# nirvanesque/headCT_foundation

Measured on AMD Instinct MI355X. Metric: CT-volumes/sec MAE pretrain step (96^3, ViT-B/16^3, mask 0.75), higher is better.
Workload: dtype bf16; 1 GPU; BASELINE config #2: MAE ViT-B/16^3, 96^3x1ch, mask 0.75, full train step (fwd+bwd+clip+AdamW+LR); per_gpu_batch=256, global_batch=256, parallelism=dp1, init=reference init, seed 42

## Files before the change

### headct_foundation_amd/_lib.py

```python
from __future__ import annotations

import ctypes as C
import os
from typing import Optional

HERE = os.path.dirname(os.path.abspath(__file__))
LIB_PATH = os.path.join(HERE, "libheadct_hip.so")

HCT_F32, HCT_BF16, HCT_F16 = 0, 1, 2
NORM_LAYERNORM, NORM_RMSNORM = 0, 1
HCT_ACT_NONE, HCT_ACT_GELU, HCT_ACT_DGELU, HCT_ACT_TANH, HCT_ACT_GELU_D, HCT_ACT_MULAUX = 0, 1, 2, 3, 4, 5
ACT_NONE, ACT_GELU, ACT_DGELU = 0, 1, 2

c_void_p, c_int, c_float, c_size_t, c_int64 = C.c_void_p, C.c_int, C.c_float, C.c_size_t, C.c_int64


class GemmArgs(C.Structure):
    _fields_ = [
        ("M", c_int), ("N", c_int), ("K", c_int),
        ("A", c_void_p), ("a_dtype", c_int), ("lda", c_int64), ("transA", c_int),
        ("B", c_void_p), ("b_dtype", c_int), ("ldb", c_int64), ("transB", c_int),
        ("C", c_void_p), ("c_dtype", c_int), ("ldc", c_int64),
        ("bias", c_void_p), ("residual", c_void_p), ("ldr", c_int64),
        ("act", c_int),
# ... 135 lines not shown
    "hct_adjust_contrast_workspace_bytes": (c_size_t, [c_int, c_int64]),
    "hct_adjust_contrast": (c_int, [c_void_p, c_int, c_int64, c_void_p, c_void_p, c_void_p, c_size_t, c_void_p]),
    "hct_volume_to_ras": (c_int, [c_void_p, c_int, c_int, c_int, c_int, C.POINTER(c_int), C.POINTER(c_int), c_int, C.c_double, C.c_double,
                                  c_void_p, c_void_p]),
    "hct_bspline3_resample_workspace_bytes": (c_size_t, [c_int] * 6),
    "hct_bspline3_resample": (c_int, [c_void_p, c_int, c_int, c_int, c_void_p, c_int, c_int, c_int, c_void_p, c_void_p, c_void_p, c_size_t, c_void_p]),
    "hct_foreground_bbox_workspace_bytes": (c_size_t, [c_int] * 3),
    "hct_foreground_bbox": (c_int, [c_void_p, c_int, c_int, c_int, c_void_p, c_void_p, c_void_p, c_size_t, c_void_p]),
    "hct_crop_window_resize_area": (c_int, [c_void_p, c_int, c_int, c_int, c_void_p, c_int, c_void_p, c_void_p, c_void_p, c_int, c_int, c_int,
                                            c_void_p]),
    "hct_pos_embed_interp3d": (c_int, [c_void_p, c_int, c_void_p, c_int, c_int, c_int, c_void_p]),
    "hct_colsum_workspace_bytes": (c_size_t, [c_int, c_int]),
    "hct_colsum": (c_int, [c_void_p, c_int, c_int, c_int, c_int64, c_void_p, c_void_p, c_size_t, c_void_p]),
    "hct_cast": (c_int, [c_void_p, c_int, c_void_p, c_int, c_int64, c_void_p]),
    "hct_transpose_cast": (c_int, [c_void_p, c_int, c_void_p, c_int, c_int, c_int, c_void_p]),
    "hct_grad_norms_workspace_bytes": (c_size_t, [c_int64]),
    "hct_grad_norms": (c_int, [c_void_p, c_void_p, c_int, c_int64, c_float, c_int, c_void_p, c_void_p, c_void_p, c_size_t, c_void_p]),
    "hct_adamw_step": (c_int, [c_void_p, c_void_p, c_void_p, c_void_p, c_void_p, c_void_p, c_void_p, c_int, c_int64, c_float, c_float,
                               c_float, c_float, c_float, c_int, c_void_p, c_void_p]),
    "hct_lion_step": (c_int, [c_void_p] * 6 + [c_int, c_int64] + [C.c_double] * 4 + [c_void_p, c_void_p]),
    "hct_sgd_step": (c_int, [c_void_p] * 6 + [c_int, c_int64] + [C.c_double] * 2 + [c_void_p, c_void_p]),
    "hct_lamb_workspace_bytes": (c_size_t, [c_int64, c_int]),
    "hct_lamb_step": (c_int, [c_void_p] * 7 + [c_int, c_int64] + [C.c_double] * 5 + [c_void_p] * 4 + [c_size_t, c_void_p, c_void_p]),
    "hct_debug_set_gemm_variant": (None, [c_int]),
    "hct_gemm_nt_stream_k_bytes": (c_size_t, []),
    "hct_gemm_tn_group_workspace_bytes": (c_size_t, [c_int]),
    "hct_gemm_tn_group_prepare": (c_int, [c_void_p, c_int, c_void_p, c_size_t, c_void_p]),
    "hct_gemm_tn_group_run": (c_int, [c_void_p, c_int, c_void_p, c_size_t, c_void_p]),
    "hct_prof_enable": (None, [c_int]),
    "hct_prof_reset": (None, []),
    "hct_prof_read": (c_int, [c_int, C.POINTER(C.c_double), C.POINTER(c_int64), C.POINTER(C.c_double)]),
    "hct_prof_read_bytes": (c_int, [c_int, C.POINTER(C.c_double)]),
    "hct_prof_shapes": (c_int, [c_int, c_void_p, c_int]),
    "hct_mae_plan_create": (c_void_p, [C.POINTER(MaeConfig), c_int, c_int]),
# ... 9 lines not shown
    "hct_mae_backward_final_offset": (c_int64, [c_void_p]),
    "hct_mae_plan_set_wgrad_defer": (c_int, [c_void_p, c_int, c_int]),
    "hct_mae_plan_set_requires_grad": (c_int, [c_void_p, c_int, c_int]),
    "hct_lora_qv_fwd": (c_int, [c_void_p, c_void_p, c_void_p, c_void_p, c_void_p, c_int, c_int, c_int, c_int, c_int, c_int, c_void_p, c_void_p, c_void_p]),
    "hct_lora_qv_bwd_workspace_bytes": (c_size_t, [c_int, c_int, c_int, c_int]),
    "hct_lora_qv_bwd": (c_int, [c_void_p] * 11 + [c_int] * 6 + [c_void_p] * 6 + [c_size_t, c_void_p]),
    "hct_topk_dot_chunks": (c_int, [c_int, c_int64]),
    "hct_topk_dot_workspace": (c_size_t, [c_int, c_int64, c_int]),
    "hct_topk_dot": (c_int, [c_void_p, c_int, c_void_p, c_int64, c_int, c_int, c_void_p, c_int, c_void_p, c_void_p, c_void_p, c_size_t, c_void_p]),
    "hct_attention_row_probs": (c_int, [c_void_p, c_int, c_int, c_int, c_int, c_int, c_void_p, c_int, c_void_p, c_void_p]),
    "hct_mae_recon_accum": (c_int, [c_void_p, c_int, c_int, c_void_p, c_int, c_void_p, c_int, c_int, c_int, c_int, c_int, c_void_p, c_void_p, c_void_p,
                                    c_void_p]),
    "hct_mae_recon_finish": (c_int, [c_void_p, c_void_p, c_void_p, c_void_p, c_int, c_int, c_int, c_int, c_int, c_void_p, c_void_p, c_void_p, c_void_p]),
    "hct_mae_plan_bind": (c_int, [c_void_p, c_void_p, c_void_p, c_void_p, c_void_p, c_void_p, c_size_t]),
    "hct_mae_refresh_weights": (c_int, [c_void_p, c_int, c_void_p]),
    "hct_mae_forward": (c_int, [c_void_p, c_void_p, c_int, c_void_p, c_void_p, c_float, c_void_p]),
    "hct_mae_set_loss_grad": (c_int, [c_void_p, c_void_p]),
    "hct_mae_num_backward_stages": (c_int, [c_void_p]),
    "hct_mae_backward_stage_range": (c_int, [c_void_p, c_int, C.POINTER(c_int64), C.POINTER(c_int64)]),
    "hct_mae_backward_stage": (c_int, [c_void_p, c_int, c_void_p]),
    "hct_vit_forward": (c_int, [c_void_p, c_void_p, c_int, c_void_p]),
    "hct_vit_forward_parts": (c_int, [c_void_p, C.POINTER(c_void_p), c_int, c_int, c_void_p]),
    "hct_vit_backward_stage": (c_int, [c_void_p, c_int, c_void_p, c_void_p]),
    "hct_vit_assemble_bwd": (c_int, [c_void_p, c_int, c_int, c_int, c_int, c_void_p, c_int, c_void_p, c_void_p, c_void_p, c_void_p]),
    "hct_mae_plan_activation": (c_void_p, [c_void_p, C.c_char_p, C.POINTER(c_int64), C.POINTER(c_int64), C.POINTER(c_int)]),
}

_lib: Optional[C.CDLL] = None


# ... 83 lines not shown
```

### headct_foundation_amd/csrc/mae_plan.hip

```cpp
#include <cstdlib>
#include "common.h"
#include "gemm_plan.h"

#include <algorithm>
#include <map>
#include <string>
#include <vector>

using namespace hct;

namespace {

constexpr int64_t kUnitElems = 1024;

struct BlockP {
  int ln1_w, ln1_b, qkv_w, qkv_b, proj_w, proj_b, ln2_w, ln2_b, fc1_w, fc1_b, fc2_w, fc2_b;
  int lq_b = -1, lq_a = -1, lv_b = -1, lv_a = -1;
  int site = 0;
};
struct BlockA {
  size_t x1, mean1, rstd1, qkv, o, lse, h_mid, x2, mean2, rstd2, u, g;
  size_t lora_t = 0;
};
struct Act { size_t off; int64_t rows, cols; int dtype; };
// ... 8 lines not shown
  int g, L, K, pd, Ne, Nd, Me, Md;
  int D, Dd, Mlp, Mlpd, H, Hd;
  std::vector<hct_param_info> params;
  std::map<std::string, int> pindex;
  int64_t param_elems = 0, bf16t_elems = 0;
  bool vit = false;
  int R = 0;
  int lora = 0;
  int norm_kind = 0;
  float drop_p = 0.f;
  bool drop_on = false;
  bool drop_fwd = false;
  uint64_t drop_seed = 0;
  size_t s_drop_y = 0;
  bool t_all_done = false;
  float norm_eps = 1e-5f;
  int p_reg = -1;
  int p_pe_w, p_pe_b, p_pos, p_cls, p_norm_w, p_norm_b, p_de_w, p_de_b, p_mask, p_dcls, p_dpos, p_dnorm_w, p_dnorm_b,
      p_pred_w, p_pred_b;
  std::vector<BlockP> enc, dec;
  std::vector<std::pair<int64_t, int64_t>> stage_range;
  size_t ws_bytes = 0;
  size_t a_ids_restore, a_ids_shuffle, a_mask, a_row_loss, a_patches, a_tok, a_latent, a_lat_mean, a_lat_rstd, a_e,
      a_ynorm, a_yn_mean, a_yn_rstd, a_pred, a_dpred;
  bool tail = false;
  bool tail_fwd = false;
  bool tail_ok = false;
  int Mc = 0;
  size_t a_tail_rows = 0, a_tail_inv = 0, a_oc = 0, s_dhc = 0;
  bool dec0 = false, dec0_fwd = false, dec0_ok = false;
// ... 799 lines not shown
}

void hct_mae_plan_destroy(hct_mae_plan* p) { delete p; }
int hct_mae_plan_num_params(const hct_mae_plan* p) { return (int)p->params.size(); }
int hct_mae_plan_param_info(const hct_mae_plan* p, int index, hct_param_info* out) {
  HCT_REQUIRE(p && out && index >= 0 && index < (int)p->params.size(), "hct_mae_plan_param_info: bad index");
  *out = p->params[index];
  return 0;
}
int64_t hct_mae_plan_param_elems(const hct_mae_plan* p) { return p->param_elems; }
int64_t hct_mae_plan_bf16_t_elems(const hct_mae_plan* p) { return p->bf16t_elems; }
size_t hct_mae_plan_workspace_bytes(const hct_mae_plan* p) { return p->ws_bytes; }
int hct_mae_plan_len_keep(const hct_mae_plan* p) { return p ? p->K : -1; }
int hct_mae_plan_set_requires_grad(hct_mae_plan* p, int index, int flag) {
  HCT_REQUIRE(p && index >= 0 && index < (int)p->params.size(), "hct_mae_plan_set_requires_grad: bad index");
  if (p->params[index].requires_grad != (flag ? 1 : 0)) p->t_all_done = false;
  p->params[index].requires_grad = flag ? 1 : 0;
  return 0;
}
int hct_mae_plan_set_dec0(hct_mae_plan* p, int on) {
  if (!p) return -1;
  p->dec0 = on != 0 && p->dec0_ok;
  return p->dec0 ? 1 : 0;
}
int hct_mae_plan_set_dropout(hct_mae_plan* p, int active, uint64_t seed) {
  if (!p) return -1;
  p->drop_on = active != 0 && p->drop_p > 0.f;
  p->drop_seed = seed;
  return p->drop_on ? 1 : 0;
}
int hct_mae_plan_set_tail(hct_mae_plan* p, int compact) {
  if (!p) return -1;
  p->tail = compact != 0 && p->tail_ok;
  return p->tail ? 1 : 0;
}

int hct_mae_plan_bind(hct_mae_plan* p, float* params, float* grads, void* params_bf16, void* params_bf16_t, void* workspace,
                      size_t workspace_bytes) {
  HCT_REQUIRE(p && params && workspace, "hct_mae_plan_bind: null buffer");
  HCT_REQUIRE(p->dt == HCT_F32 || (params_bf16 && params_bf16_t), "hct_mae_plan_bind: bf16 mode needs the bf16 weight buffers");
  if (workspace_bytes < p->ws_bytes) { set_error("hct_mae_plan_bind: workspace too small"); return HCT_E_WORKSPACE; }
  p->params_f32 = params; p->grads = grads;
  p->params_bf16 = (bf16*)params_bf16; p->params_bf16_t = (bf16*)params_bf16_t;
  p->ws = (unsigned char*)workspace;
  p->nt_ws_armed = false;
  p->t_all_done = false;
  p->fwd_done = false;
  for (auto& v : p->wg_prepared) v.clear();
  p->wg_pending.clear();
  return 0;
}

int hct_mae_refresh_weights(hct_mae_plan* p, int with_plain, void* stream) {
  HCT_REQUIRE(p && p->params_f32, "hct_mae_refresh_weights: plan not bound");
  if (p->dt != HCT_BF16) return 0;
  if (with_plain) RC(hct_cast(p->params_f32, HCT_F32, p->params_bf16, HCT_BF16, p->param_elems, stream));
  TransposeTable t;
  t.n = 0;
  t.tile_start[0] = 0;
  auto flush = [&]() -> int {
    if (t.n == 0) return 0;
    hipLaunchKernelGGL(transpose_cast_batched_kernel, dim3(t.tile_start[t.n]), dim3(256), 0, (hipStream_t)stream, p->params_f32,
                       p->params_bf16_t, t);
    t.n = 0;
    return check_hip(hipGetLastError(), "hct_mae_refresh_weights");
  };
  for (const auto& pi : p->params) {
    if (pi.bf16_t_offset < 0) continue;
    if (!with_plain && p->t_all_done && !pi.requires_grad) continue;
    const int rows = (int)pi.shape[0], cols = (int)(pi.numel / pi.shape[0]);
    t.rows[t.n] = rows; t.cols[t.n] = cols; t.src[t.n] = pi.offset; t.dst[t.n] = pi.bf16_t_offset;
    t.tile_start[t.n + 1] = t.tile_start[t.n] + ((rows + 63) / 64) * ((cols + 63) / 64);
    if (++t.n == kMaxT) RC(flush());
  }
  RC(flush());
  p->t_all_done = true;
  return 0;
}

int hct_mae_forward(hct_mae_plan* p, const void* x, int x_dtype, const float* noise, float* loss, float grad_scale, void* stream) {
  HCT_REQUIRE(p && p->ws && x && noise && loss, "hct_mae_forward: plan not bound or null argument");
  HCT_REQUIRE(!p->vit, "hct_mae_forward: encoder-only plans are driven by hct_vit_forward");
  HCT_REQUIRE(x_dtype == HCT_F32 || x_dtype == HCT_F16, "hct_mae_forward: volumes are fp32 or fp16");
  hipStream_t s = (hipStream_t)stream;
  unsigned char* ws = p->ws;
  const hct_mae_config& c = p->cfg;
  const int B = p->B;
  int32_t* ids_restore = (int32_t*)(ws + p->a_ids_restore);
  int32_t* ids_shuffle = (int32_t*)(ws + p->a_ids_shuffle);
  float* mask = (float*)(ws + p->a_mask);
// ... 213 lines not shown
```

### headct_foundation_amd/csrc/optim.hip

```cpp
#include "common.h"

namespace hct {

constexpr int kUnit = 1024;

__device__ __forceinline__ float block_sum_256(float v, float* s_tmp) {
  v = wave_sum(v);
  __syncthreads();
  if ((threadIdx.x & 63) == 0) s_tmp[threadIdx.x >> 6] = v;
  __syncthreads();
  return (s_tmp[0] + s_tmp[1]) + (s_tmp[2] + s_tmp[3]);
}

__global__ void __launch_bounds__(256) sumsq_units_kernel(const float* __restrict__ g, int64_t total,
                                                          float* __restrict__ unit_sumsq) {
  __shared__ float s_tmp[4];
  const int64_t i = (int64_t)blockIdx.x * kUnit + threadIdx.x * 4;
  float s = 0.f;
  if (i < total) {
    const f32x4 v = Vec4<float>::load(g + i);
    s = (v[0] * v[0] + v[1] * v[1]) + (v[2] * v[2] + v[3] * v[3]);
  }
  s = block_sum_256(s, s_tmp);
  if (threadIdx.x == 0) unit_sumsq[blockIdx.x] = s;
// ... 33 lines not shown
  const int64_t base = (int64_t)blockIdx.x * kUnit;
  const float c = coef[find_segment(seg_off, nseg, base)];
  if (c == 1.0f) return;
  const int64_t i = base + threadIdx.x * 4;
  if (i < total) Vec4<float>::store(g + i, Vec4<float>::load(g + i) * c);
}

struct AdamArgs {
  float lr_wd_keep;
  float one_m_b1, b2, one_m_b2;
  float step_size;
  float inv_bc2_sqrt;
  float eps;
};

__global__ void __launch_bounds__(256) adamw_units_kernel(float* __restrict__ p, float* __restrict__ g, float* __restrict__ m,
                                                          float* __restrict__ v, const int64_t* __restrict__ seg_off,
                                                          const float* __restrict__ coef, const uint8_t* __restrict__ skip,
                                                          int nseg, int64_t total, AdamArgs a, bf16* __restrict__ p_bf16) {
  const int64_t base = (int64_t)blockIdx.x * kUnit;
  const int sgi = find_segment(seg_off, nseg, base);
  const int64_t i = base + threadIdx.x * 4;
  if (i >= total) return;
  if (skip && skip[sgi]) return;
  const float c = coef ? coef[sgi] : 1.0f;
  f32x4 gv = Vec4<float>::load_nt(g + i);
  if (c != 1.0f) {
    gv = gv * c;
    Vec4<float>::store(g + i, gv);
  }
  f32x4 pv = Vec4<float>::load_nt(p + i) * a.lr_wd_keep;
  f32x4 mv = Vec4<float>::load_nt(m + i);
  mv = mv + (gv - mv) * a.one_m_b1;
  f32x4 vv = Vec4<float>::load_nt(v + i) * a.b2 + gv * gv * a.one_m_b2;
  f32x4 den;
#pragma unroll
  for (int e = 0; e < 4; ++e) den[e] = sqrtf(vv[e]) * a.inv_bc2_sqrt + a.eps;
#pragma unroll
  for (int e = 0; e < 4; ++e) pv[e] = pv[e] - a.step_size * (mv[e] / den[e]);
  Vec4<float>::store_nt(p + i, pv);
  Vec4<float>::store_nt(m + i, mv);
  Vec4<float>::store_nt(v + i, vv);
  if (p_bf16) Vec4<bf16>::store(p_bf16 + i, pv);
}

struct LionArgs {
  float lr_wd_keep;
  float lr, b1, one_m_b1, b2, one_m_b2;
};

__global__ void __launch_bounds__(256) lion_units_kernel(float* __restrict__ p, float* __restrict__ g, float* __restrict__ m,
                                                         const int64_t* __restrict__ seg_off, const float* __restrict__ coef,
                                                         const uint8_t* __restrict__ skip, int nseg, int64_t total, LionArgs a,
                                                         bf16* __restrict__ p_bf16) {
  const int64_t base = (int64_t)blockIdx.x * kUnit;
  const int sgi = find_segment(seg_off, nseg, base);
  const int64_t i = base + threadIdx.x * 4;
  if (i >= total) return;
// ... 141 lines not shown
  HCT_REQUIRE(total > 0 && total % kUnit == 0 && nseg > 0, "hct_grad_norms: total must be a positive multiple of %d", kUnit);
  if (workspace_bytes < hct_grad_norms_workspace_bytes(total)) {
    set_error("hct_grad_norms: workspace too small");
    return HCT_E_WORKSPACE;
  }
  hipStream_t s = (hipStream_t)stream;
  const int units = (int)(total / kUnit);
  hipLaunchKernelGGL(sumsq_units_kernel, dim3(units), dim3(256), 0, s, grads, total, (float*)workspace);
  hipLaunchKernelGGL(seg_norm_kernel, dim3(nseg), dim3(256), 0, s, (const float*)workspace, seg_off, clip, norms, coef);
  if (scale_in_place && clip > 0.f)
    hipLaunchKernelGGL(scale_units_kernel, dim3(units), dim3(256), 0, s, grads, seg_off, coef, nseg, total);
  HCT_CHECK_LAUNCH("hct_grad_norms");
  return 0;
}

int hct_adamw_step(float* params, float* grads, float* exp_avg, float* exp_avg_sq, const int64_t* seg_off,
                   const float* coef, const uint8_t* skip, int nseg, int64_t total, float lr, float beta1, float beta2,
                   float eps, float weight_decay, int step, void* params_bf16, void* stream) {
  HCT_REQUIRE(total > 0 && total % kUnit == 0 && nseg > 0 && step >= 1, "hct_adamw_step: bad arguments");
  AdamArgs a;
  const double bc1 = 1.0 - pow((double)beta1, (double)step);
  const double bc2 = 1.0 - pow((double)beta2, (double)step);
  a.lr_wd_keep = (float)(1.0 - (double)lr * (double)weight_decay);
  a.one_m_b1 = (float)(1.0 - (double)beta1);
  a.b2 = beta2;
  a.one_m_b2 = (float)(1.0 - (double)beta2);
  a.step_size = (float)((double)lr / bc1);
  a.inv_bc2_sqrt = (float)(1.0 / sqrt(bc2));
  a.eps = eps;
  hipLaunchKernelGGL(adamw_units_kernel, dim3((int)(total / kUnit)), dim3(256), 0, (hipStream_t)stream, params, grads,
                     exp_avg, exp_avg_sq, seg_off, coef, skip, nseg, total, a, (bf16*)params_bf16);
  HCT_CHECK_LAUNCH("hct_adamw_step");
  return 0;
}

int hct_lion_step(float* params, float* grads, float* exp_avg, const int64_t* seg_off, const float* coef, const uint8_t* skip,
                  int nseg, int64_t total, double lr, double beta1, double beta2, double weight_decay, void* params_bf16,
                  void* stream) {
  HCT_REQUIRE(params && grads && exp_avg && seg_off && total > 0 && total % kUnit == 0 && nseg > 0, "hct_lion_step: bad arguments");
  LionArgs a;
  a.lr_wd_keep = (float)(1.0 - lr * weight_decay);
  a.lr = (float)lr;
  a.b1 = (float)beta1;
  a.one_m_b1 = (float)(1.0 - beta1);
  a.b2 = (float)beta2;
  a.one_m_b2 = (float)(1.0 - beta2);
  hipLaunchKernelGGL(lion_units_kernel, dim3((int)(total / kUnit)), dim3(256), 0, (hipStream_t)stream, params, grads, exp_avg,
// ... 54 lines not shown
```

### headct_foundation_amd/flat.py

```python
from __future__ import annotations

import ctypes as C
from typing import Callable, Dict, List, Optional, Tuple

import torch
import torch.nn as nn

from . import _lib
from ._lib import HCT_BF16, HctError


class FlatModule(nn.Module):

    def _init_flat(self) -> None:
        self._weights_version = 0
        self._managed_updates = False
        self._grad_prescale = 1.0
        self._build_flat(torch.device("cpu"))

    def _flat_layout(self) -> Tuple[List[Tuple[str, int, int, Tuple[int, ...], bool, int]], int]:
        layout, off = [], 0
        for n, p in self.named_parameters():
            layout.append((n, off, p.numel(), tuple(p.shape), bool(p.requires_grad), -1))
            off += (p.numel() + 1023) // 1024 * 1024
# ... 137 lines not shown
        for name, off, numel, shape, rg, _ in self._layout:
            p = self._named_cache[name]
            p.requires_grad_(rg and p.requires_grad)
            g = old_grads[name]
            if g is not None:
                self._flat_grad[off:off + numel].copy_(g.reshape(-1))
                p.grad = self._flat_grad[off:off + numel].view(shape)
        if self._dt == HCT_BF16:
            self._flat_bf16 = torch.zeros(total, dtype=torch.bfloat16, device=device)
            self._flat_bf16_t = torch.zeros(max(self._bf16_t_elems, 1), dtype=torch.bfloat16, device=device)
        else:
            self._flat_bf16 = self._flat_bf16_t = None
        self._plans = {}
        self._plain_fresh = False

    def mark_weights_updated(self, plain_bf16_fresh: bool = False) -> None:
        super().mark_weights_updated()
        self._plain_fresh = plain_bf16_fresh

    def _init_dropout(self, dropout_rate: float) -> None:
        self.dropout_rate = float(dropout_rate)
        self.last_dropout_seed: Optional[int] = None
        self._next_dropout_seed: Optional[int] = None

    def set_dropout_seed(self, seed: int) -> None:
        self._next_dropout_seed = int(seed) & 0xFFFFFFFFFFFFFFFF

    def _arm_dropout(self, plan: _Plan) -> bool:
        rate = getattr(self, "dropout_rate", 0.0)
        active = bool(self.training and rate > 0.0)
        seed = 0
        if active:
            if self._next_dropout_seed is not None:
# ... 102 lines not shown
```

### headct_foundation_amd/optim.py

```python
from __future__ import annotations

from itertools import chain
from typing import List, Optional

import torch

from . import _lib
from ._lib import HctError
from .flat import FlatModule
from .mae import MaskedAutoencoderViT


def unwrap(model):
    while hasattr(model, "module") and not isinstance(model, FlatModule):
        model = model.module
    return model


class _FlatState:

    def __init__(self, model):
        self.model = model
        self.flat_id = None
        self.refresh()
# ... 2 lines not shown
        m = self.model
        dev = m._flat.device
        names, seg = m.flat_segments()
        self.names = names
        self.nseg = len(names)
        self.total = seg[-1]
        self.seg_off = torch.tensor(seg, dtype=torch.int64, device=dev)
        named = dict(m.named_parameters())
        self.skip = torch.tensor([0 if named[n].requires_grad else 1 for n in names], dtype=torch.uint8, device=dev)
        self.norms = torch.zeros(self.nseg, dtype=torch.float32, device=dev)
        self.coef = torch.ones(self.nseg, dtype=torch.float32, device=dev)
        lib = _lib.load()
        self.ws = torch.empty(max(16, lib.hct_grad_norms_workspace_bytes(self.total)), dtype=torch.uint8, device=dev)
        self.flat_id = m._flat.data_ptr()
        self.coef_pending = False

    def ensure(self):
        if self.flat_id != self.model._flat.data_ptr():
            self.refresh()


def _state_for(model) -> _FlatState:
    st = getattr(model, "_flat_state", None)
    if st is None:
        st = _FlatState(model)
        model._flat_state = st
    st.ensure()
    return st


# ... 126 lines not shown
        m = self._model
        if not m._flat.is_cuda:
            raise HctError(f"{type(self).__name__}.step needs the model on a GPU; there is no CPU fallback")
        self._ensure_state()
        st = _state_for(m)
        grp = self.param_groups[0]
        self._step_count_fused += 1
        lib = _lib.load()
        coef = st.coef.data_ptr() if st.coef_pending else None
        named = getattr(m, "_named_cache", None) or dict(m.named_parameters())
        key = tuple((not named[n].requires_grad) or named[n].grad is None for n in st.names)
        if getattr(st, "skip_key", None) != key:
            st.skip = torch.tensor([1 if k else 0 for k in key], dtype=torch.uint8, device=m._flat.device)
            st.skip_key = key
        self._skipped = dict(zip(st.names, key))
        self._launch(lib, m, st, grp, coef)
        st.coef_pending = False
        self._after_launch()
        m.mark_weights_updated(plain_bf16_fresh=m._flat_bf16 is not None)
        return loss


class HipAdamW(_FlatOptimizer):

    _BUFFERS = ("exp_avg", "exp_avg_sq")

    def __init__(self, model, lr=1e-3, betas=(0.9, 0.999), eps=1e-8, weight_decay=1e-2):
        defaults = dict(lr=lr, betas=betas, eps=eps, weight_decay=weight_decay, amsgrad=False, maximize=False,
                        foreach=None, capturable=False, differentiable=False, fused=None, decoupled_weight_decay=True)
        self._step_tensor = torch.tensor(0.0)
        super().__init__(model, defaults)

    def _entry(self, views, seg, prev):
        return {"step": self._step_tensor, **views}

    def _after_load(self):
        self._step_tensor = torch.tensor(float(self._step_count_fused))

    def _launch(self, lib, m, st, grp, coef):
        _lib.check(lib.hct_adamw_step(
            m._flat.data_ptr(), m._flat_grad.data_ptr(), self._flat_buffer("exp_avg").data_ptr(), self._flat_buffer("exp_avg_sq").data_ptr(),
            st.seg_off.data_ptr(), coef, st.skip.data_ptr(), st.nseg, st.total, float(grp["lr"]), float(grp["betas"][0]),
            float(grp["betas"][1]), float(grp["eps"]), float(grp["weight_decay"]), self._step_count_fused,
            _lib.ptr(m._flat_bf16), _lib.stream_ptr()), "hct_adamw_step")

    def _after_launch(self):
        self._step_tensor.fill_(float(self._step_count_fused))


class HipLion(_FlatOptimizer):

    _BUFFERS = ("exp_avg",)

    def __init__(self, model, lr=1e-4, betas=(0.9, 0.99), weight_decay=0.0):
        assert lr > 0.0 and all(0.0 <= b <= 1.0 for b in betas), f"HipLion needs lr > 0 and betas in [0, 1]: got lr={lr}, betas={betas}"
        super().__init__(model, dict(lr=lr, betas=betas, weight_decay=weight_decay))

    def _launch(self, lib, m, st, grp, coef):
        _lib.check(lib.hct_lion_step(
# ... 93 lines not shown
```

### include/headct_hip.h

```cpp
#ifndef HEADCT_HIP_H
#define HEADCT_HIP_H

#include <stddef.h>
#include <stdint.h>

#ifdef __cplusplus
extern "C" {
#endif

#define HCT_F32 0
#define HCT_BF16 1
#define HCT_F16 2

#define HCT_E_BADARG (-1)
#define HCT_E_UNSUPPORTED (-2)
#define HCT_E_WORKSPACE (-3)
#define HCT_E_STATE (-4)

#define HCT_ACT_NONE 0
#define HCT_ACT_GELU 1
#define HCT_ACT_DGELU 2
#define HCT_ACT_TANH 3
#define HCT_ACT_GELU_D 4
#define HCT_ACT_MULAUX 5
// ... 192 lines not shown
int hct_bspline3_resample(const float* in, int n0, int n1, int n2, float* out, int m0, int m1, int m2, const int32_t* base, const double* weights,
                          void* workspace, size_t workspace_bytes, void* stream);
size_t hct_foreground_bbox_workspace_bytes(int m0, int m1, int m2);
int hct_foreground_bbox(const float* vol, int m0, int m1, int m2, int32_t* box, int32_t* status, void* workspace, size_t workspace_bytes, void* stream);
int hct_crop_window_resize_area(const float* vol, int m0, int m1, int m2, const int32_t* box, int n_windows, const float* a_min, const float* a_max,
                                void* out, int R0, int R1, int R2, void* stream);

int hct_pos_embed_interp3d(const float* src, int g_src, float* dst, int g_dst, int D, int extra, void* stream);

size_t hct_colsum_workspace_bytes(int rows, int cols);
int hct_colsum(const void* x, int dtype, int rows, int cols, int64_t ld, float* out, void* workspace,
               size_t workspace_bytes, void* stream);

int hct_cast(const void* src, int src_dtype, void* dst, int dst_dtype, int64_t n, void* stream);
int hct_transpose_cast(const void* src, int src_dtype, void* dst, int dst_dtype, int rows, int cols, void* stream);

size_t hct_grad_norms_workspace_bytes(int64_t total);
int hct_grad_norms(float* grads, const int64_t* seg_off, int nseg, int64_t total, float clip, int scale_in_place,
                   float* norms, float* coef, void* workspace, size_t workspace_bytes, void* stream);
int hct_adamw_step(float* params, float* grads, float* exp_avg, float* exp_avg_sq, const int64_t* seg_off,
                   const float* coef, const uint8_t* skip, int nseg, int64_t total, float lr, float beta1,
                   float beta2, float eps, float weight_decay, int step, void* params_bf16, void* stream);
int hct_lion_step(float* params, float* grads, float* exp_avg, const int64_t* seg_off, const float* coef,
                  const uint8_t* skip, int nseg, int64_t total, double lr, double beta1, double beta2, double weight_decay,
                  void* params_bf16, void* stream);
int hct_sgd_step(float* params, float* grads, float* momentum_buf, const int64_t* seg_off, const float* coef,
                 const uint8_t* skip, int nseg, int64_t total, double lr, double momentum, void* params_bf16, void* stream);
size_t hct_lamb_workspace_bytes(int64_t total, int nseg);
int hct_lamb_step(float* params, float* grads, float* exp_avg, float* exp_avg_sq, const int64_t* seg_off, const float* coef,
                  const uint8_t* skip, int nseg, int64_t total, double lr, double beta1, double beta2, double eps,
                  double weight_decay, float* weight_norm, float* adam_norm, float* trust_ratio, void* workspace,
                  size_t workspace_bytes, void* params_bf16, void* stream);

typedef struct hct_mae_config {
  int input_size, patch_size, in_chans;
  double mask_ratio;
  int pos_embed;
// ... 22 lines not shown

hct_mae_plan* hct_mae_plan_create(const hct_mae_config* cfg, int batch, int compute_dtype);
void hct_mae_plan_destroy(hct_mae_plan*);
int hct_mae_plan_num_params(const hct_mae_plan*);
int hct_mae_plan_param_info(const hct_mae_plan*, int index, hct_param_info* out);
int64_t hct_mae_plan_param_elems(const hct_mae_plan*);
int64_t hct_mae_plan_bf16_t_elems(const hct_mae_plan*);
size_t hct_mae_plan_workspace_bytes(const hct_mae_plan*);
int hct_mae_plan_len_keep(const hct_mae_plan*);
int hct_mae_plan_set_tail(hct_mae_plan*, int compact);
int hct_mae_plan_set_dec0(hct_mae_plan*, int on);
int hct_mae_plan_set_dropout(hct_mae_plan*, int active, uint64_t seed);
int hct_mae_plan_bind(hct_mae_plan*, float* params, float* grads, void* params_bf16, void* params_bf16_t,
                      void* workspace, size_t workspace_bytes);
int hct_mae_refresh_weights(hct_mae_plan*, int with_plain, void* stream);
int hct_mae_forward(hct_mae_plan*, const void* x, int x_dtype, const float* noise, float* loss, float grad_scale, void* stream);
int hct_mae_set_loss_grad(hct_mae_plan*, const float* dloss);
int hct_mae_num_backward_stages(const hct_mae_plan*);
int hct_mae_backward_stage_range(const hct_mae_plan*, int stage, int64_t* begin, int64_t* end);
int hct_mae_backward_stage(hct_mae_plan*, int stage, void* stream);
int64_t hct_mae_backward_final_offset(const hct_mae_plan*);
int hct_mae_plan_set_wgrad_defer(hct_mae_plan*, int defer, int group_blocks);
int hct_mae_plan_set_requires_grad(hct_mae_plan*, int index, int flag);
int hct_vit_forward(hct_mae_plan*, const void* x, int x_dtype, void* stream);
int hct_vit_forward_parts(hct_mae_plan*, const void* const* xs, int n_parts, int x_dtype, void* stream);
int hct_vit_backward_stage(hct_mae_plan*, int stage, const void* dlatent, void* stream);
int hct_vit_assemble_bwd(const float* dh0, int B, int L, int R, int D, void* dtok, int dtok_dtype, float* dcls, float* dreg, float* dpos,
                         void* stream);
int hct_lora_qv_fwd(const void* x1, const void* Aq, const void* Av, const void* Bq, const void* Bv, int B, int N, int H, int dh, int r, int dtype,
                    void* T, void* qkv, void* stream);
// ... 33 lines not shown
```

Measured before the change: 7089 CT-volumes/s.

## Fuse transposed bf16 weight cast into AdamW step for matrix parameters

Adds a tiled AdamW kernel that updates each weight matrix and, in the same pass, writes the transposed bf16 copy through shared memory. Non-matrix units still go through the flat unit kernel via an index list. The plan is told the transposed copy is fresh, so the next refresh_weights skips its separate transpose-cast pass. This removes one full read of the fp32 parameters plus a kernel launch per step, at the cost of more complex, less coalesced optimizer tiles and an extra freshness flag that has to stay consistent.

```diff
diff --git a/headct_foundation_amd/_lib.py b/headct_foundation_amd/_lib.py
--- a/headct_foundation_amd/_lib.py
+++ b/headct_foundation_amd/_lib.py
@@ -173,10 +173,14 @@
     "hct_colsum": (c_int, [c_void_p, c_int, c_int, c_int, c_int64, c_void_p, c_void_p, c_size_t, c_void_p]),
     "hct_cast": (c_int, [c_void_p, c_int, c_void_p, c_int, c_int64, c_void_p]),
     "hct_transpose_cast": (c_int, [c_void_p, c_int, c_void_p, c_int, c_int, c_int, c_void_p]),
+    "hct_transpose_cast_batched": (c_int, [c_void_p, c_void_p, c_void_p, c_int, c_void_p]),
     "hct_grad_norms_workspace_bytes": (c_size_t, [c_int64]),
     "hct_grad_norms": (c_int, [c_void_p, c_void_p, c_int, c_int64, c_float, c_int, c_void_p, c_void_p, c_void_p, c_size_t, c_void_p]),
     "hct_adamw_step": (c_int, [c_void_p, c_void_p, c_void_p, c_void_p, c_void_p, c_void_p, c_void_p, c_int, c_int64, c_float, c_float,
                                c_float, c_float, c_float, c_int, c_void_p, c_void_p]),
+    "hct_adamw_step_transposed": (c_int, [c_void_p, c_void_p, c_void_p, c_void_p, c_void_p, c_void_p, c_void_p, c_int, c_int64, c_float,
+                                          c_float, c_float, c_float, c_float, c_int, c_void_p, c_void_p, c_int64, c_void_p, c_int,
+                                          c_void_p, c_int, c_void_p]),
     "hct_lion_step": (c_int, [c_void_p] * 6 + [c_int, c_int64] + [C.c_double] * 4 + [c_void_p, c_void_p]),
     "hct_sgd_step": (c_int, [c_void_p] * 6 + [c_int, c_int64] + [C.c_double] * 2 + [c_void_p, c_void_p]),
     "hct_lamb_workspace_bytes": (c_size_t, [c_int64, c_int]),
@@ -216,6 +220,7 @@
     "hct_mae_recon_finish": (c_int, [c_void_p, c_void_p, c_void_p, c_void_p, c_int, c_int, c_int, c_int, c_int, c_void_p, c_void_p, c_void_p, c_void_p]),
     "hct_mae_plan_bind": (c_int, [c_void_p, c_void_p, c_void_p, c_void_p, c_void_p, c_void_p, c_size_t]),
     "hct_mae_refresh_weights": (c_int, [c_void_p, c_int, c_void_p]),
+    "hct_mae_plan_set_transposed_fresh": (c_int, [c_void_p, c_int]),
     "hct_mae_forward": (c_int, [c_void_p, c_void_p, c_int, c_void_p, c_void_p, c_float, c_void_p]),
     "hct_mae_set_loss_grad": (c_int, [c_void_p, c_void_p]),
     "hct_mae_num_backward_stages": (c_int, [c_void_p]),
diff --git a/headct_foundation_amd/csrc/mae_plan.hip b/headct_foundation_amd/csrc/mae_plan.hip
--- a/headct_foundation_amd/csrc/mae_plan.hip
+++ b/headct_foundation_amd/csrc/mae_plan.hip
@@ -46,6 +46,7 @@
   uint64_t drop_seed = 0;
   size_t s_drop_y = 0;
   bool t_all_done = false;
+  bool t_fresh = false;
   float norm_eps = 1e-5f;
   int p_reg = -1;
   int p_pe_w, p_pe_b, p_pos, p_cls, p_norm_w, p_norm_b, p_de_w, p_de_b, p_mask, p_dcls, p_dpos, p_dnorm_w, p_dnorm_b,
@@ -875,7 +876,7 @@
 int hct_mae_plan_len_keep(const hct_mae_plan* p) { return p ? p->K : -1; }
 int hct_mae_plan_set_requires_grad(hct_mae_plan* p, int index, int flag) {
   HCT_REQUIRE(p && index >= 0 && index < (int)p->params.size(), "hct_mae_plan_set_requires_grad: bad index");
-  if (p->params[index].requires_grad != (flag ? 1 : 0)) p->t_all_done = false;
+  if (p->params[index].requires_grad != (flag ? 1 : 0)) p->t_all_done = p->t_fresh = false;
   p->params[index].requires_grad = flag ? 1 : 0;
   return 0;
 }
@@ -905,36 +906,56 @@
   p->params_bf16 = (bf16*)params_bf16; p->params_bf16_t = (bf16*)params_bf16_t;
   p->ws = (unsigned char*)workspace;
   p->nt_ws_armed = false;
-  p->t_all_done = false;
+  p->t_all_done = p->t_fresh = false;
   p->fwd_done = false;
   for (auto& v : p->wg_prepared) v.clear();
   p->wg_pending.clear();
   return 0;
 }
 
-int hct_mae_refresh_weights(hct_mae_plan* p, int with_plain, void* stream) {
-  HCT_REQUIRE(p && p->params_f32, "hct_mae_refresh_weights: plan not bound");
-  if (p->dt != HCT_BF16) return 0;
-  if (with_plain) RC(hct_cast(p->params_f32, HCT_F32, p->params_bf16, HCT_BF16, p->param_elems, stream));
+int hct_transpose_cast_batched(const float* src, void* dst_bf16, const int64_t* mats, int nmat, void* stream) {
+  HCT_REQUIRE(src && dst_bf16 && mats && nmat >= 0, "hct_transpose_cast_batched: null argument");
   TransposeTable t;
   t.n = 0;
   t.tile_start[0] = 0;
   auto flush = [&]() -> int {
     if (t.n == 0) return 0;
-    hipLaunchKernelGGL(transpose_cast_batched_kernel, dim3(t.tile_start[t.n]), dim3(256), 0, (hipStream_t)stream, p->params_f32,
-                       p->params_bf16_t, t);
+    hipLaunchKernelGGL(transpose_cast_batched_kernel, dim3(t.tile_start[t.n]), dim3(256), 0, (hipStream_t)stream, src, (bf16*)dst_bf16, t);
     t.n = 0;
-    return check_hip(hipGetLastError(), "hct_mae_refresh_weights");
+    return check_hip(hipGetLastError(), "hct_transpose_cast_batched");
   };
+  for (int i = 0; i < nmat; ++i) {
+    const int64_t off = mats[4 * i], rows = mats[4 * i + 1], cols = mats[4 * i + 2], t_off = mats[4 * i + 3];
+    HCT_REQUIRE(off >= 0 && t_off >= 0 && rows > 0 && cols > 0 && rows < (1 << 24) && cols < (1 << 24),
+                "hct_transpose_cast_batched: bad matrix %d", i);
+    t.rows[t.n] = (int)rows; t.cols[t.n] = (int)cols; t.src[t.n] = off; t.dst[t.n] = t_off;
+    t.tile_start[t.n + 1] = t.tile_start[t.n] + (int)(((rows + 63) / 64) * ((cols + 63) / 64));
+    if (++t.n == kMaxT) RC(flush());
+  }
+  return flush();
+}
+
+int hct_mae_plan_set_transposed_fresh(hct_mae_plan* p, int fresh) {
+  if (!p) return -1;
+  p->t_fresh = fresh != 0 && p->dt == HCT_BF16 && p->t_all_done;
+  return p->t_fresh ? 1 : 0;
+}
+
+int hct_mae_refresh_weights(hct_mae_plan* p, int with_plain, void* stream) {
+  HCT_REQUIRE(p && p->params_f32, "hct_mae_refresh_weights: plan not bound");
+  if (p->dt != HCT_BF16) return 0;
+  const bool fresh = p->t_fresh;
+  p->t_fresh = false;
+  if (!with_plain && fresh) return 0;
+  if (with_plain) RC(hct_cast(p->params_f32, HCT_F32, p->params_bf16, HCT_BF16, p->param_elems, stream));
+  std::vector<int64_t> mats;
   for (const auto& pi : p->params) {
     if (pi.bf16_t_offset < 0) continue;
     if (!with_plain && p->t_all_done && !pi.requires_grad) continue;
-    const int rows = (int)pi.shape[0], cols = (int)(pi.numel / pi.shape[0]);
-    t.rows[t.n] = rows; t.cols[t.n] = cols; t.src[t.n] = pi.offset; t.dst[t.n] = pi.bf16_t_offset;
-    t.tile_start[t.n + 1] = t.tile_start[t.n] + ((rows + 63) / 64) * ((cols + 63) / 64);
-    if (++t.n == kMaxT) RC(flush());
-  }
-  RC(flush());
+    const int64_t rows = pi.shape[0], cols = pi.numel / pi.shape[0];
+    mats.insert(mats.end(), {pi.offset, rows, cols, pi.bf16_t_offset});
+  }
+  RC(hct_transpose_cast_batched(p->params_f32, p->params_bf16_t, mats.data(), (int)(mats.size() / 4), stream));
   p->t_all_done = true;
   return 0;
 }
diff --git a/headct_foundation_amd/csrc/optim.hip b/headct_foundation_amd/csrc/optim.hip
--- a/headct_foundation_amd/csrc/optim.hip
+++ b/headct_foundation_amd/csrc/optim.hip
@@ -71,11 +71,30 @@
   float eps;
 };
 
+__device__ __forceinline__ void adamw_update4(f32x4& pv, const f32x4& gv, f32x4& mv, f32x4& vv, const AdamArgs& a) {
+  pv = pv * a.lr_wd_keep;
+  mv = mv + (gv - mv) * a.one_m_b1;
+  vv = vv * a.b2 + gv * gv * a.one_m_b2;
+  f32x4 den;
+#pragma unroll
+  for (int e = 0; e < 4; ++e) den[e] = sqrtf(vv[e]) * a.inv_bc2_sqrt + a.eps;
+#pragma unroll
+  for (int e = 0; e < 4; ++e) pv[e] = pv[e] - a.step_size * (mv[e] / den[e]);
+}
+__device__ __forceinline__ void adamw_update1(float& pv, float gv, float& mv, float& vv, const AdamArgs& a) {
+  pv = pv * a.lr_wd_keep;
+  mv = mv + (gv - mv) * a.one_m_b1;
+  vv = vv * a.b2 + gv * gv * a.one_m_b2;
+  const float den = sqrtf(vv) * a.inv_bc2_sqrt + a.eps;
+  pv = pv - a.step_size * (mv / den);
+}
+
 __global__ void __launch_bounds__(256) adamw_units_kernel(float* __restrict__ p, float* __restrict__ g, float* __restrict__ m,
                                                           float* __restrict__ v, const int64_t* __restrict__ seg_off,
                                                           const float* __restrict__ coef, const uint8_t* __restrict__ skip,
-                                                          int nseg, int64_t total, AdamArgs a, bf16* __restrict__ p_bf16) {
-  const int64_t base = (int64_t)blockIdx.x * kUnit;
+                                                          int nseg, int64_t total, AdamArgs a, bf16* __restrict__ p_bf16,
+                                                          const int32_t* __restrict__ unit_list) {
+  const int64_t base = (int64_t)(unit_list ? unit_list[blockIdx.x] : (int32_t)blockIdx.x) * kUnit;
   const int sgi = find_segment(seg_off, nseg, base);
   const int64_t i = base + threadIdx.x * 4;
   if (i >= total) return;
@@ -86,19 +105,124 @@
     gv = gv * c;
     Vec4<float>::store(g + i, gv);
   }
-  f32x4 pv = Vec4<float>::load_nt(p + i) * a.lr_wd_keep;
+  f32x4 pv = Vec4<float>::load_nt(p + i);
   f32x4 mv = Vec4<float>::load_nt(m + i);
-  mv = mv + (gv - mv) * a.one_m_b1;
-  f32x4 vv = Vec4<float>::load_nt(v + i) * a.b2 + gv * gv * a.one_m_b2;
-  f32x4 den;
-#pragma unroll
-  for (int e = 0; e < 4; ++e) den[e] = sqrtf(vv[e]) * a.inv_bc2_sqrt + a.eps;
-#pragma unroll
-  for (int e = 0; e < 4; ++e) pv[e] = pv[e] - a.step_size * (mv[e] / den[e]);
+  f32x4 vv = Vec4<float>::load_nt(v + i);
+  adamw_update4(pv, gv, mv, vv, a);
   Vec4<float>::store_nt(p + i, pv);
   Vec4<float>::store_nt(m + i, mv);
   Vec4<float>::store_nt(v + i, vv);
   if (p_bf16) Vec4<bf16>::store(p_bf16 + i, pv);
+}
+
+constexpr int kMaxTiled = 96;
+struct AdamTileTable {
+  int n;
+  int tile_start[kMaxTiled + 1];
+  int rows[kMaxTiled], cols[kMaxTiled], seg[kMaxTiled];
+  long long off[kMaxTiled], t_off[kMaxTiled];
+};
+
+__global__ void __launch_bounds__(256) adamw_tiles_kernel(float* __restrict__ p, float* __restrict__ g, float* __restrict__ m,
+                                                          float* __restrict__ v, const float* __restrict__ coef,
+                                                          const uint8_t* __restrict__ skip, AdamArgs a, bf16* __restrict__ p_bf16,
+                                                          bf16* __restrict__ p_bf16_t, AdamTileTable t) {
+  constexpr int TC = 64, G = 4;
+  constexpr int LR = TC / 4, RS = 256 / LR, NIT = 64 / RS;
+  __shared__ float tile[64][TC + 1];
+  int lo = 0, hi = t.n;
+  while (hi - lo > 1) {
+    const int mid = (lo + hi) >> 1;
+    if (t.tile_start[mid] <= (int)blockIdx.x) lo = mid; else hi = mid;
+  }
+  const int sgi = t.seg[lo];
+  if (skip && skip[sgi]) return;
+  const float c = coef ? coef[sgi] : 1.0f;
+  const int rows = t.rows[lo], cols = t.cols[lo];
+  const int local = blockIdx.x - t.tile_start[lo];
+  const int tcols = (cols + TC - 1) / TC;
+  const int r0 = (local / tcols) * 64, c0 = (local % tcols) * TC;
+  const int64_t base = t.off[lo];
+  bf16* __restrict__ d = p_bf16_t + t.t_off[lo];
+  if ((cols & 3) == 0) {
+    const int q = threadIdx.x % LR, rr = threadIdx.x / LR;
+    const int cc = c0 + q * 4;
+#pragma unroll
+    for (int i0 = 0; i0 < NIT; i0 += G) {
+      f32x4 gv[G], pv[G], mv[G], vv[G];
+      bool ok[G];
+#pragma unroll
+      for (int i = 0; i < G; ++i) {
+        const int r = r0 + rr + RS * (i0 + i);
+        ok[i] = r < rows && cc < cols;
+        const int64_t e = base + (int64_t)r * cols + cc;
+        gv[i] = pv[i] = mv[i] = vv[i] = f32x4{0.f, 0.f, 0.f, 0.f};
+        if (ok[i]) {
+          gv[i] = Vec4<float>::load_nt(g + e);
+          pv[i] = Vec4<float>::load_nt(p + e);
+          mv[i] = Vec4<float>::load_nt(m + e);
+          vv[i] = Vec4<float>::load_nt(v + e);
+        }
+      }
+#pragma unroll
+      for (int i = 0; i < G; ++i) {
+        if (ok[i]) {
+          const int64_t e = base + (int64_t)(r0 + rr + RS * (i0 + i)) * cols + cc;
+          if (c != 1.0f) {
+            gv[i] = gv[i] * c;
+            Vec4<float>::store(g + e, gv[i]);
+          }
+          adamw_update4(pv[i], gv[i], mv[i], vv[i], a);
+          Vec4<float>::store_nt(p + e, pv[i]);
+          Vec4<float>::store_nt(m + e, mv[i]);
+          Vec4<float>::store_nt(v + e, vv[i]);
+          if (p_bf16) Vec4<bf16>::store(p_bf16 + e, pv[i]);
+        }
+#pragma unroll
+        for (int k = 0; k < 4; ++k) tile[rr + RS * (i0 + i)][q * 4 + k] = pv[i][k];
+      }
+    }
+  } else {
+    const int tx = threadIdx.x % TC, ty = threadIdx.x / TC;
+    for (int i = ty; i < 64; i += 256 / TC) {
+      const int r = r0 + i, cc = c0 + tx;
+      float pv = 0.f;
+      if (r < rows && cc < cols) {
+        const int64_t e = base + (int64_t)r * cols + cc;
+        float gv = __builtin_nontemporal_load(g + e);
+        if (c != 1.0f) {
+          gv = gv * c;
+          g[e] = gv;
+        }
+        pv = __builtin_nontemporal_load(p + e);
+        float mv = __builtin_nontemporal_load(m + e), vv = __builtin_nontemporal_load(v + e);
+        adamw_update1(pv, gv, mv, vv, a);
+        __builtin_nontemporal_store(pv, p + e);
+        __builtin_nontemporal_store(mv, m + e);
+        __builtin_nontemporal_store(vv, v + e);
+        if (p_bf16) p_bf16[e] = (bf16)pv;
+      }
+      tile[i][tx] = pv;
+    }
+  }
+  __syncthreads();
+  if ((rows & 3) == 0) {
+    const int q = threadIdx.x & 15, rr = threadIdx.x >> 4;
+#pragma unroll
+    for (int i = 0; i < TC / 16; ++i) {
+      const int cc = c0 + rr + 16 * i, r = r0 + q * 4;
+      if (cc < cols && r < rows) {
+        const f32x4 o = {tile[q * 4 + 0][rr + 16 * i], tile[q * 4 + 1][rr + 16 * i], tile[q * 4 + 2][rr + 16 * i], tile[q * 4 + 3][rr + 16 * i]};
+        Vec4<bf16>::store(d + (int64_t)cc * rows + r, o);
+      }
+    }
+  } else {
+    const int tx = threadIdx.x & 63, ty = threadIdx.x >> 6;
+    for (int i = ty; i < TC; i += 4) {
+      const int cc = c0 + i, r = r0 + tx;
+      if (cc < cols && r < rows) d[(int64_t)cc * rows + r] = (bf16)tile[tx][i];
+    }
+  }
 }
 
 struct LionArgs {
@@ -270,10 +394,7 @@
   return 0;
 }
 
-int hct_adamw_step(float* params, float* grads, float* exp_avg, float* exp_avg_sq, const int64_t* seg_off,
-                   const float* coef, const uint8_t* skip, int nseg, int64_t total, float lr, float beta1, float beta2,
-                   float eps, float weight_decay, int step, void* params_bf16, void* stream) {
-  HCT_REQUIRE(total > 0 && total % kUnit == 0 && nseg > 0 && step >= 1, "hct_adamw_step: bad arguments");
+static AdamArgs adam_args(float lr, float beta1, float beta2, float eps, float weight_decay, int step) {
   AdamArgs a;
   const double bc1 = 1.0 - pow((double)beta1, (double)step);
   const double bc2 = 1.0 - pow((double)beta2, (double)step);
@@ -284,9 +405,59 @@
   a.step_size = (float)((double)lr / bc1);
   a.inv_bc2_sqrt = (float)(1.0 / sqrt(bc2));
   a.eps = eps;
+  return a;
+}
+
+int hct_adamw_step(float* params, float* grads, float* exp_avg, float* exp_avg_sq, const int64_t* seg_off,
+                   const float* coef, const uint8_t* skip, int nseg, int64_t total, float lr, float beta1, float beta2,
+                   float eps, float weight_decay, int step, void* params_bf16, void* stream) {
+  HCT_REQUIRE(total > 0 && total % kUnit == 0 && nseg > 0 && step >= 1, "hct_adamw_step: bad arguments");
+  const AdamArgs a = adam_args(lr, beta1, beta2, eps, weight_decay, step);
   hipLaunchKernelGGL(adamw_units_kernel, dim3((int)(total / kUnit)), dim3(256), 0, (hipStream_t)stream, params, grads,
-                     exp_avg, exp_avg_sq, seg_off, coef, skip, nseg, total, a, (bf16*)params_bf16);
+                     exp_avg, exp_avg_sq, seg_off, coef, skip, nseg, total, a, (bf16*)params_bf16, (const int32_t*)nullptr);
   HCT_CHECK_LAUNCH("hct_adamw_step");
+  return 0;
+}
+
+int hct_adamw_step_transposed(float* params, float* grads, float* exp_avg, float* exp_avg_sq, const int64_t* seg_off,
+                              const float* coef, const uint8_t* skip, int nseg, int64_t total, float lr, float beta1, float beta2,
+                              float eps, float weight_decay, int step, void* params_bf16, void* params_bf16_t, int64_t bf16_t_elems,
+                              const int64_t* mats, int nmat, const int32_t* rest_units, int n_rest, void* stream) {
+  HCT_REQUIRE(params && grads && exp_avg && exp_avg_sq && seg_off && total > 0 && total % kUnit == 0 && nseg > 0 && step >= 1,
+              "hct_adamw_step_transposed: bad arguments");
+  HCT_REQUIRE(params_bf16_t && mats && nmat > 0 && n_rest >= 0 && (n_rest == 0 || rest_units) && n_rest <= total / kUnit,
+              "hct_adamw_step_transposed: needs the transposed buffer, a matrix table and the list of the remaining units");
+  for (int i = 0; i < nmat; ++i) {
+    const int64_t sg = mats[5 * i], off = mats[5 * i + 1], rows = mats[5 * i + 2], cols = mats[5 * i + 3], t_off = mats[5 * i + 4];
+    HCT_REQUIRE(sg >= 0 && sg < nseg && rows > 0 && cols > 0 && rows < (1 << 24) && cols < (1 << 24) && off >= 0 && off % kUnit == 0 &&
+                    off + rows * cols <= total && t_off >= 0 && t_off % 64 == 0 && t_off + rows * cols <= bf16_t_elems,
+                "hct_adamw_step_transposed: matrix %d (segment %lld, %lld x %lld at %lld, transposed at %lld) does not fit its buffers", i,
+                (long long)sg, (long long)rows, (long long)cols, (long long)off, (long long)t_off);
+  }
+  const AdamArgs a = adam_args(lr, beta1, beta2, eps, weight_decay, step);
+  hipStream_t s = (hipStream_t)stream;
+  if (n_rest > 0)
+    hipLaunchKernelGGL(adamw_units_kernel, dim3(n_rest), dim3(256), 0, s, params, grads, exp_avg, exp_avg_sq, seg_off, coef, skip, nseg,
+                       total, a, (bf16*)params_bf16, rest_units);
+  AdamTileTable t;
+  t.n = 0;
+  t.tile_start[0] = 0;
+  auto flush = [&]() {
+    if (t.n == 0) return;
+    hipLaunchKernelGGL(adamw_tiles_kernel, dim3(t.tile_start[t.n]), dim3(256), 0, s, params, grads, exp_avg, exp_avg_sq, coef, skip, a,
+                       (bf16*)params_bf16, (bf16*)params_bf16_t, t);
+    t.n = 0;
+  };
+  for (int i = 0; i < nmat; ++i) {
+    const int rows = (int)mats[5 * i + 2], cols = (int)mats[5 * i + 3];
+    const int64_t tiles = (int64_t)((rows + 63) / 64) * ((cols + 63) / 64);
+    if (t.n == kMaxTiled || t.tile_start[t.n] + tiles > (int64_t)1 << 30) flush();
+    t.seg[t.n] = (int)mats[5 * i]; t.off[t.n] = mats[5 * i + 1]; t.rows[t.n] = rows; t.cols[t.n] = cols; t.t_off[t.n] = mats[5 * i + 4];
+    t.tile_start[t.n + 1] = t.tile_start[t.n] + (int)tiles;
+    ++t.n;
+  }
+  flush();
+  HCT_CHECK_LAUNCH("hct_adamw_step_transposed");
   return 0;
 }
 
diff --git a/headct_foundation_amd/flat.py b/headct_foundation_amd/flat.py
--- a/headct_foundation_amd/flat.py
+++ b/headct_foundation_amd/flat.py
@@ -175,9 +175,11 @@
         self._plans = {}
         self._plain_fresh = False
 
-    def mark_weights_updated(self, plain_bf16_fresh: bool = False) -> None:
+    def mark_weights_updated(self, plain_bf16_fresh: bool = False, transposed_fresh: bool = False) -> None:
         super().mark_weights_updated()
         self._plain_fresh = plain_bf16_fresh
+        for plan in self._plans.values():
+            plan.lib.hct_mae_plan_set_transposed_fresh(plan.handle, int(transposed_fresh and plain_bf16_fresh))
 
     def _init_dropout(self, dropout_rate: float) -> None:
         self.dropout_rate = float(dropout_rate)
diff --git a/headct_foundation_amd/optim.py b/headct_foundation_amd/optim.py
--- a/headct_foundation_amd/optim.py
+++ b/headct_foundation_amd/optim.py
@@ -40,6 +40,23 @@
         self.ws = torch.empty(max(16, lib.hct_grad_norms_workspace_bytes(self.total)), dtype=torch.uint8, device=dev)
         self.flat_id = m._flat.data_ptr()
         self.coef_pending = False
+        self._transposed_tables(m, names, seg, dev)
+
+    def _transposed_tables(self, m, names, seg, dev):
+        import ctypes as C
+        self.t_mats, self.t_nmat, self.t_rest = None, 0, None
+        if getattr(m, "_flat_bf16_t", None) is None:
+            return
+        index = {n: i for i, n in enumerate(names)}
+        rows = [(index[n], off, shape[0], numel // shape[0], t_off) for n, off, numel, shape, _, t_off in m._layout if t_off >= 0]
+        if not rows:
+            return
+        self.t_nmat = len(rows)
+        self.t_mats = (C.c_int64 * (5 * len(rows)))(*[v for r in rows for v in r])
+        tiled = torch.zeros(self.total // 1024, dtype=torch.bool)
+        for i, *_ in rows:
+            tiled[seg[i] // 1024:seg[i + 1] // 1024] = True
+        self.t_rest = torch.nonzero(~tiled).flatten().to(dtype=torch.int32, device=dev)
 
     def ensure(self):
         if self.flat_id != self.model._flat.data_ptr():
@@ -196,10 +213,14 @@
             st.skip = torch.tensor([1 if k else 0 for k in key], dtype=torch.uint8, device=m._flat.device)
             st.skip_key = key
         self._skipped = dict(zip(st.names, key))
+        self._wrote_transposed = False
         self._launch(lib, m, st, grp, coef)
         st.coef_pending = False
         self._after_launch()
-        m.mark_weights_updated(plain_bf16_fresh=m._flat_bf16 is not None)
+        if self._wrote_transposed:
+            m.mark_weights_updated(plain_bf16_fresh=True, transposed_fresh=True)
+        else:
+            m.mark_weights_updated(plain_bf16_fresh=m._flat_bf16 is not None)
         return loss
 
 
@@ -220,11 +241,15 @@
         self._step_tensor = torch.tensor(float(self._step_count_fused))
 
     def _launch(self, lib, m, st, grp, coef):
-        _lib.check(lib.hct_adamw_step(
-            m._flat.data_ptr(), m._flat_grad.data_ptr(), self._flat_buffer("exp_avg").data_ptr(), self._flat_buffer("exp_avg_sq").data_ptr(),
-            st.seg_off.data_ptr(), coef, st.skip.data_ptr(), st.nseg, st.total, float(grp["lr"]), float(grp["betas"][0]),
-            float(grp["betas"][1]), float(grp["eps"]), float(grp["weight_decay"]), self._step_count_fused,
-            _lib.ptr(m._flat_bf16), _lib.stream_ptr()), "hct_adamw_step")
+        head = (m._flat.data_ptr(), m._flat_grad.data_ptr(), self._flat_buffer("exp_avg").data_ptr(), self._flat_buffer("exp_avg_sq").data_ptr(),
+                st.seg_off.data_ptr(), coef, st.skip.data_ptr(), st.nseg, st.total, float(grp["lr"]), float(grp["betas"][0]),
+                float(grp["betas"][1]), float(grp["eps"]), float(grp["weight_decay"]), self._step_count_fused, _lib.ptr(m._flat_bf16))
+        if st.t_nmat:
+            _lib.check(lib.hct_adamw_step_transposed(*head, m._flat_bf16_t.data_ptr(), m._flat_bf16_t.numel(), st.t_mats, st.t_nmat,
+                                                     st.t_rest.data_ptr(), st.t_rest.numel(), _lib.stream_ptr()), "hct_adamw_step_transposed")
+            self._wrote_transposed = True
+        else:
+            _lib.check(lib.hct_adamw_step(*head, _lib.stream_ptr()), "hct_adamw_step")
 
     def _after_launch(self):
         self._step_tensor.fill_(float(self._step_count_fused))
diff --git a/include/headct_hip.h b/include/headct_hip.h
--- a/include/headct_hip.h
+++ b/include/headct_hip.h
@@ -230,6 +230,7 @@
 
 int hct_cast(const void* src, int src_dtype, void* dst, int dst_dtype, int64_t n, void* stream);
 int hct_transpose_cast(const void* src, int src_dtype, void* dst, int dst_dtype, int rows, int cols, void* stream);
+int hct_transpose_cast_batched(const float* src, void* dst_bf16, const int64_t* mats, int nmat, void* stream);
 
 size_t hct_grad_norms_workspace_bytes(int64_t total);
 int hct_grad_norms(float* grads, const int64_t* seg_off, int nseg, int64_t total, float clip, int scale_in_place,
@@ -237,6 +238,11 @@
 int hct_adamw_step(float* params, float* grads, float* exp_avg, float* exp_avg_sq, const int64_t* seg_off,
                    const float* coef, const uint8_t* skip, int nseg, int64_t total, float lr, float beta1,
                    float beta2, float eps, float weight_decay, int step, void* params_bf16, void* stream);
+int hct_adamw_step_transposed(float* params, float* grads, float* exp_avg, float* exp_avg_sq, const int64_t* seg_off,
+                              const float* coef, const uint8_t* skip, int nseg, int64_t total, float lr, float beta1,
+                              float beta2, float eps, float weight_decay, int step, void* params_bf16, void* params_bf16_t,
+                              int64_t bf16_t_elems, const int64_t* mats, int nmat, const int32_t* rest_units, int n_rest,
+                              void* stream);
 int hct_lion_step(float* params, float* grads, float* exp_avg, const int64_t* seg_off, const float* coef,
                   const uint8_t* skip, int nseg, int64_t total, double lr, double beta1, double beta2, double weight_decay,
                   void* params_bf16, void* stream);
@@ -289,6 +295,7 @@
 int hct_mae_plan_bind(hct_mae_plan*, float* params, float* grads, void* params_bf16, void* params_bf16_t,
                       void* workspace, size_t workspace_bytes);
 int hct_mae_refresh_weights(hct_mae_plan*, int with_plain, void* stream);
+int hct_mae_plan_set_transposed_fresh(hct_mae_plan*, int fresh);
 int hct_mae_forward(hct_mae_plan*, const void* x, int x_dtype, const float* noise, float* loss, float grad_scale, void* stream);
 int hct_mae_set_loss_grad(hct_mae_plan*, const float* dloss);
 int hct_mae_num_backward_stages(const hct_mae_plan*);
```

Result: no change. 7102 CT-volumes/s, median of 5 (+0.2%).
